# josl/kmerjs

Measured on AMD Instinct MI355X. Metric: k-mers/sec + distinct-kmers/sec, k=16 150bp synthetic FASTQ, 1/2/4/8 GPU, higher is better.
Workload: dtype u8; 1 GPU; C2: 10000000 synthetic 150bp reads per GPU, k=16, prefix 'ATGAC'; reads_per_gpu=10000000, mode=ordered (reference Map insertion order), k=16, prefix=ATGAC, bytes_per_gpu=3170000000, pipeline=off (steps in sequence), parallelism=dp1 (one GPU; no collective), backend=none

## Files before the change

kmerjs_amd/csrc/kmer_kernels.hip:

```cpp
#include "kmer_device.hpp"

#include <algorithm>
#include <cstring>

namespace kmerhip {

__device__ __forceinline__ uint32_t align4(uint32_t hi, uint32_t lo, uint32_t sel) {
    return __builtin_amdgcn_alignbyte(hi, lo, sel);
}

__device__ __forceinline__ void set_info(unsigned int *err, unsigned int bit) {
    if (!(__hip_atomic_load(err, __ATOMIC_RELAXED, __HIP_MEMORY_SCOPE_AGENT) & bit)) atomicOr(err, bit);
}

__device__ __forceinline__ uint32_t not_nl_bits(uint32_t x) {
    return ((x ^ 0x0A0A0A0Au) + 0x7F7F7F7Fu) & 0x80808080u;
}

__device__ __forceinline__ uint32_t not_nl_bits_xad(uint32_t x, uint32_t k0a, uint32_t k7f) {
    uint32_t r;
    asm("v_xad_u32 %0, %1, %2, %3" : "=v"(r) : "v"(x), "v"(k0a), "s"(k7f));
    return r & 0x80808080u;
}

// ... 41 lines not shown
            if (incmask) return acc;
        } else {
            unsigned long long hit = __ballot(inc || val != 0);
            if (hit) {
                int stop = __ffsll((long long)hit) - 1;
                return __shfl(val, stop);
            }
        }
        top -= 64;
    }
}

struct TileShared {
    uint32_t tpre[TPB + 1];
    uint32_t wsum[TPB / 64];
    int32_t last_thr;
    uint32_t tile;
    uint64_t line_base;
    uint64_t lnl_before;
    uint64_t lnl_tile;
    int32_t lastpos;
    uint32_t nh;
    uint32_t qn;
    uint32_t more;
    uint32_t q[1024];
};

__device__ __forceinline__ uint32_t nl_before_in_thread(const uint8_t *buf, int thr, int q) {
    const uint32_t *lw = (const uint32_t *)(buf + FH + 64 * thr);
    int n = q - 64 * thr;
    uint32_t c = 0;
#pragma unroll 1
    for (int i = 0; i < 16 && n > 0; ++i, n -= 4) {
        uint32_t z = nl_flags(lw[i]);
        if (n < 4) z &= (1u << (8 * n)) - 1u;
        c += __popc(z);
    }
    return c;
}

__device__ __forceinline__ uint32_t lds_word(const uint8_t *buf, int p) {
    const int a = FH + p;
    const uint32_t *w = (const uint32_t *)(buf + (a & ~3));
    return align4(w[1], w[0], (uint32_t)(a & 3));
}


__device__ __forceinline__ uint64_t revcomp_code(uint64_t x, uint32_t k) {
    x = ~x;
    x = ((x >> 2) & 0x3333333333333333ull) | ((x & 0x3333333333333333ull) << 2);
    x = ((x >> 4) & 0x0F0F0F0F0F0F0F0Full) | ((x & 0x0F0F0F0F0F0F0F0Full) << 4);
    x = __builtin_bswap64(x);
    return k >= 32 ? x : (x >> (64 - 2 * k));
}

__device__ __forceinline__ void revcomp_code128(uint64_t hi, uint64_t lo, uint32_t k, uint64_t *rhi, uint64_t *rlo) {
    const uint64_t h = revcomp_code(lo, 32), l = revcomp_code(hi, 32);
    const uint32_t s = 128 - 2 * k;
    *rlo = s ? (l >> s) | (h << (64 - s)) : l;
    *rhi = s ? h >> s : h;
}

__device__ __forceinline__ uint32_t tile_prologue(const uint8_t *data, uint64_t len, int64_t g0, uint8_t *buf,
                                                  TileShared &sh, uint32_t (&w)[17], unsigned int *err) {
    const int tid = threadIdx.x, lane = tid & 63, wid = tid >> 6;
    TileRegs r;
    load_tile(data, len, g0, r);
    if (store_tile(r, buf) & 0x80808080u) atomicOr(err, ERR_NONASCII);
    __syncthreads();

    load_thread_words(buf + FH + 64 * tid, w);
    uint32_t cnt = 0;
    const int64_t gt = g0 + 64 * tid;
    if (gt + 64 <= (int64_t)len) {
#pragma unroll
        for (int i = 0; i < 16; ++i) cnt += __popc(nl_flags(w[i]));
    } else {
#pragma unroll
        for (int i = 0; i < 16; ++i) cnt += __popc(nl_flags_below(w[i], (int64_t)len - (gt + 4 * i)));
    }
    uint32_t incl = cnt;
#pragma unroll
    for (int d = 1; d < 64; d <<= 1) {
        const uint32_t y = __shfl_up(incl, d);
        if (lane >= d) incl += y;
    }
    if (lane == 63) sh.wsum[wid] = incl;
    if (cnt) atomicMax(&sh.last_thr, tid);
    __syncthreads();
    uint32_t woff = 0, total = 0;
#pragma unroll
    for (int i = 0; i < TPB / 64; ++i) {
        woff += i < wid ? sh.wsum[i] : 0;
        total += sh.wsum[i];
    }
    sh.tpre[tid] = woff + incl - cnt;
    if (tid == 0) sh.tpre[TPB] = total;
    if (tid == sh.last_thr) {
        int lastpos = -1;
#pragma unroll 1
        for (int i = 15; i >= 0 && lastpos < 0; --i) {
            const uint32_t z = nl_flags_below(*(const uint32_t *)(buf + FH + 64 * tid + 4 * i),
                                              (int64_t)len - (gt + 4 * i));
            if (z) lastpos = 64 * tid + 4 * i + ((31 - __clz(z)) >> 3);
        }
        sh.lastpos = lastpos;
// ... 620 lines not shown
    uint32_t wpre[TPB / 64], wprev[TPB / 64], tcnt = 0, tlast = 0;
    {
        const uint4 ws = *(const uint4 *)sh.wsum, wm = *(const uint4 *)sh.wmax;
        const uint32_t s[4] = {ws.x, ws.y, ws.z, ws.w}, m[4] = {wm.x, wm.y, wm.z, wm.w};
#pragma unroll
        for (int ww = 0; ww < TPB / 64; ++ww) {
            wpre[ww] = tcnt;
            wprev[ww] = tlast;
            tcnt += (uint32_t)__builtin_amdgcn_readfirstlane((int)s[ww]);
            tlast = max(tlast, (uint32_t)__builtin_amdgcn_readfirstlane((int)m[ww]));
        }
    }
    if (tid == 0) {
        a.tsum[tile].cnt = tcnt;
        a.tsum[tile].lnl = tlast ? a.abs_offset + (uint64_t)(g0 + tlast) : 0;
        sh.tcnt = tcnt;
    }
    for (uint32_t done = 0;;) {
        const uint32_t left = total - done;
        uint2 en = make_uint2(0u, 0u);
        if ((uint32_t)tid < min(left, QE)) en = qe[tid];
        const uint32_t nc = __popc(en.y), incl = wave_incl_sum(nc);
        const uint32_t wtot = readlane32(incl, 63);
        uint32_t *flat = sh.flat[wid & 1];
        for (uint32_t cb = 0; cb < wtot; cb += 64) {
            uint32_t m = en.y, p = incl - nc - cb;
            while (m) {
                const uint32_t bit = __ffs(m) - 1;
                m &= m - 1;
                if (p < 64) flat[p] = (en.x + (bit << 1)) | ((uint32_t)tid << 16);
                ++p;
            }
            if ((uint32_t)lane < min(wtot - cb, 64u)) {
                const uint32_t f = flat[lane], ow = (f >> 13) & 3u;
                uint4 lc = sh.qc[f >> 16];
                const uint32_t wp = ow == 0 ? wpre[0] : ow == 1 ? wpre[1] : ow == 2 ? wpre[2] : wpre[3];
                const uint32_t wl = ow == 0 ? wprev[0] : ow == 1 ? wprev[1] : ow == 2 ? wprev[2] : wprev[3];
                const uint32_t prv = lc.x >> 16;
                lc.x = (lc.x & 0xFFFFu) + wp;
                lc.w = prv ? prv : wl;
                emit_hit<true, WIDE, K, PLEN>(a, buf, sh, tile, f & 0xFFFFu, pb, pw, lc, tcnt);
            }
        }
        if (left <= QE) break;
        __syncthreads();
        done += QE;
        enqueue(done);
        __syncthreads();
    }
    if (total > 64) __syncthreads();
    if (tid == 0) put_tile_hits(a, sh, tile);
}

__device__ __forceinline__ uint64_t resolve_hit(const HitArgs &a, uint64_t pos_lines, const HitRec &r,
                                                uint64_t code_hi, const TileSum &tb, uint64_t *order_out,
                                                uint32_t *lk, bool *lvalid_out, uint64_t *key_hi) {
    const uint32_t t = r.tile;
    const uint32_t strand = (r.qm >> 14) & 1u;
    const bool exotic = (r.qm >> 15) & 1u;
    const bool lvalid = (r.qm >> 16) & 1u;
    const int q = (int)(r.qm & 0x3FFFu);
    const int s0 = strand ? q + (int)a.plen - (int)a.k : q;
    const uint64_t tile_abs = a.abs_offset + (uint64_t)t * TILE;
    const uint64_t li = pos_lines + tb.cnt + r.c_local;
    const uint64_t lstart = lvalid ? tile_abs + r.lstart : tb.lnl;
    const uint64_t sabs = tile_abs + (uint64_t)(int64_t)s0;
    uint64_t rel = sabs - lstart;
    const bool seq = (li & 3) == 1;
    const uint64_t maxrel = (1ull << a.pbits) - 1ull;
    if (rel > maxrel) {
        if (seq) atomicOr(a.err, ERR_LINE_TOO_LONG);
        rel = maxrel;
    }
    if (li >> (63 - a.pbits)) atomicOr(a.err, ERR_LINE_TOO_LONG);
    const uint64_t order = (li << (a.pbits + 1)) | ((uint64_t)strand << a.pbits) | (strand ? maxrel - rel : rel);
    *order_out = order;
    const uint32_t sp = (uint32_t)(s0 + 64);
    *lk = (r.c_local << 17) | (strand << 16) | (strand ? 0xFFFFu - sp : sp);
    *lvalid_out = lvalid;
    uint64_t key = a.invalid_key;
    *key_hi = a.wide ? a.invalid_key : 0;
    if (a.wide) key = 0;
    if (seq) {
        if (a.packed && !exotic) {
            if (a.k > 32) {
                uint64_t h = code_hi, l = r.code;
                if (strand) revcomp_code128(code_hi, r.code, a.k, &h, &l);
                key = l & a.smask;
                *key_hi = h & a.smask_hi;
            } else {
                key = (strand ? revcomp_code(r.code, a.k) : r.code) & a.smask;
            }
        } else {
            append_record(a.recs, a.rec_count, a.rec_cap, a.err, order, (uint64_t)t * TILE + (uint64_t)(int64_t)s0, a.k,
                          strand);
        }
    }
    return key;
}

__device__ __forceinline__ void place_hit(const HitArgs &a, uint64_t slot, bool cross, uint64_t xi, uint64_t key,
                                          uint64_t key_hi, uint64_t order) {
    if (!cross) {
        if (slot >= a.rcap) {
            atomicOr(a.err, ERR_OVF_OVERFLOW);
            return;
        }
        if (a.rkey32) a.rkey32[slot] = (uint32_t)key;
        else a.rkey[slot] = key;
        if (a.wide) a.rkeyh[slot] = key_hi;
        a.rord[slot] = order;
    } else if (xi < a.xcap) {
        a.xord[xi] = order;
        a.xslot[xi] = (uint32_t)slot;
        if (a.wide) {
            a.xkey[xi] = xi;
            a.xkeyl[xi] = key;
            a.xkeyh[xi] = key_hi;
        } else {
            a.xkey[xi] = key;
        }
    } else {
        atomicOr(a.err, ERR_CROSS_OVERFLOW);
    }
}

constexpr uint32_t HTPW = 4;
constexpr uint32_t HENT = HTPW * HMAX;
template <bool WIDE>
__global__ __launch_bounds__(256) void hit_kernel(HitArgs a) {
    __shared__ uint32_t s_lk[4][HENT];
    __shared__ uint8_t s_x[4][HENT];
    __shared__ uint64_t s_key[4][HENT];
    __shared__ uint64_t s_ord[4][HENT];
    __shared__ uint64_t s_keyh[WIDE ? 4 : 1][WIDE ? HENT : 1];
    const uint32_t wid = threadIdx.x >> 6, lane = threadIdx.x & 63;
    const uint32_t t0 = __builtin_amdgcn_readfirstlane((blockIdx.x * 4 + wid) * HTPW);
    if (t0 >= a.n_tiles) return;
    const unsigned long long ovf = *a.ovf_count;
    const uint64_t pos_lines = a.pos->lines;
    TileSum ts[HTPW], tb[HTPW];
#pragma unroll
    for (uint32_t u = 0; u < HTPW; ++u) {
        const uint32_t t = min(t0 + u, a.n_tiles - 1);
        ts[u] = a.tsum[t];
        tb[u] = a.tscan[t];
    }
    if (ovf > a.ovf_cap) return;
    uint32_t off[HTPW + 1];
    off[0] = 0;
#pragma unroll
    for (uint32_t u = 0; u < HTPW; ++u) off[u + 1] = off[u] + (t0 + u < a.n_tiles ? min(ts[u].nh, (uint32_t)HMAX) : 0u);
    const uint32_t total = off[HTPW];
    for (uint32_t e0 = 0; e0 < total; e0 += 64) {
        const uint32_t e = e0 + lane;
        if (e < total) {
            uint32_t u = 0;
#pragma unroll
            for (uint32_t v = 1; v < HTPW; ++v) u += e >= off[v] ? 1u : 0u;
            const uint32_t i = e - off[u];
            TileSum tsu = ts[0], tbu = tb[0];
#pragma unroll
            for (uint32_t v = 1; v < HTPW; ++v)
                if (u == v) {
                    tsu = ts[v];
                    tbu = tb[v];
                }
            const uint64_t hslot = (uint64_t)(t0 + u) * HMAX + i;
            const HitRec r = a.hits[hslot];
            uint64_t order, kh;
            uint32_t lk;
            bool lvalid;
            const uint64_t key = resolve_hit(a, pos_lines, r, a.k > 32 ? a.hits_hi[hslot] : 0, tbu, &order, &lk, &lvalid,
                                             &kh);
            s_lk[wid][e] = lk;
            s_x[wid][e] = (tsu.nh > (uint32_t)HMAX || !lvalid || r.c_local == (uint32_t)tsu.cnt) ? 1 : 0;
            s_key[wid][e] = key;
            if (WIDE) s_keyh[WIDE ? wid : 0][WIDE ? e : 0] = kh;
            s_ord[wid][e] = order;
        }
    }
    if (!a.packed) return;
    __builtin_amdgcn_fence(__ATOMIC_RELEASE, "workgroup");
    __builtin_amdgcn_wave_barrier();
    for (uint32_t e0 = 0; e0 < total; e0 += 64) {
        const uint32_t e = e0 + lane;
        if (e >= total) continue;
        uint32_t u = 0;
#pragma unroll
        for (uint32_t v = 1; v < HTPW; ++v) u += e >= off[v] ? 1u : 0u;
        uint32_t lo = off[0], hi = off[1], nh = ts[0].nh;
        uint64_t hb = tb[0].nh, xb = tb[0].nx;
#pragma unroll
        for (uint32_t v = 1; v < HTPW; ++v)
            if (u == v) {
                lo = off[v];
                hi = off[v + 1];
                nh = ts[v].nh;
                hb = tb[v].nh;
                xb = tb[v].nx;
            }
        const uint32_t i = e - lo;
        const bool cross = s_x[wid][e] != 0;
        uint32_t rank = i, xr = i;
        if (nh <= (uint32_t)HMAX) {
            const uint32_t lk = s_lk[wid][e];
            rank = 0;
            xr = 0;
            for (uint32_t j = lo; j < hi; ++j) {
                const uint32_t less = s_lk[wid][j] < lk ? 1u : 0u;
                rank += less;
                xr += less & (uint32_t)s_x[wid][j];
            }
        }
        place_hit(a, a.out_base + hb + rank, cross, a.xbase + xb + xr, s_key[wid][e],
                  WIDE ? s_keyh[WIDE ? wid : 0][WIDE ? e : 0] : 0, s_ord[wid][e]);
    }
}

__global__ __launch_bounds__(256) void hit_overflow_kernel(HitArgs a) {
    const uint64_t n = *a.ovf_count <= a.ovf_cap ? *a.ovf_count : 0;
    for (uint64_t i = (uint64_t)blockIdx.x * blockDim.x + threadIdx.x; i < n; i += (uint64_t)gridDim.x * blockDim.x) {
        const HitRec r = a.ovf[i];
        const TileSum tb = a.tscan[r.tile];
        uint64_t order, kh;
        uint32_t lk;
        bool lvalid;
        const uint64_t key = resolve_hit(a, a.pos->lines, r, a.k > 32 ? a.ovf_hi[i] : 0, tb, &order, &lk, &lvalid, &kh);
        if (!a.packed) continue;
        const uint32_t ord = r.qm >> 17;
        place_hit(a, a.out_base + tb.nh + ord, true, a.xbase + tb.nx + ord, key, kh, order);
    }
    __shared__ bool last;
    __syncthreads();
    if (threadIdx.x == 0) {
        __threadfence();
        last = atomicAdd(a.ticket, 1u) == gridDim.x - 1;
    }
    __syncthreads();
    if (!last || threadIdx.x != 0) return;
    __threadfence();
    const uint32_t nt = a.n_tiles;
    StreamPos *pos = (StreamPos *)a.pos;
    pos->lines += a.tscan[nt - 1].cnt + a.tsum[nt - 1].cnt;
    pos->ends_open = (a.len > 0 && a.data[a.len - 1] != '\n') ? 1 : 0;
    *a.ends_open = pos->ends_open;
    *a.chunk_hits = a.tscan[nt - 1].nh + a.tsum[nt - 1].nh;
    *a.chunk_cross = a.tscan[nt - 1].nx + a.tsum[nt - 1].nx;
    *a.ticket = 0;
    if (a.stamp) a.stamp[STAMP_FEED_END] = wall_clock64();
    const uint64_t errw = __hip_atomic_load(a.scal + 5, __ATOMIC_RELAXED, __HIP_MEMORY_SCOPE_AGENT);
    *a.cross_go = ((uint32_t)errw & CROSS_HOST_BITS) ? 0u : 1u;
    __threadfence();
    if (a.host_out) {
        for (int i = 0; i < 8; ++i)
            a.host_out[i] = i == 5 ? errw : __hip_atomic_load(a.scal + i, __ATOMIC_RELAXED, __HIP_MEMORY_SCOPE_AGENT);
        if (a.stamp)
            for (int i = 0; i <= (int)STAMP_FEED_END; ++i)
                a.host_out[TAIL_STAMP + i] = __hip_atomic_load(a.stamp + i, __ATOMIC_RELAXED, __HIP_MEMORY_SCOPE_AGENT);
        __threadfence_system();
        __hip_atomic_store(a.host_out + 9, a.seq, __ATOMIC_RELEASE, __HIP_MEMORY_SCOPE_SYSTEM);
    }
}

__device__ __forceinline__ TileSum ts_shfl_up(const TileSum &v, int d) {
    TileSum r;
    r.cnt = (uint64_t)__shfl_up((unsigned long long)v.cnt, d);
    r.nh = (uint32_t)__shfl_up((int)v.nh, d);
    r.nx = (uint32_t)__shfl_up((int)v.nx, d);
    r.lnl = (uint64_t)__shfl_up((unsigned long long)v.lnl, d);
    return r;
}
__device__ __forceinline__ TileSum ts_zero() {
    TileSum z;
    z.cnt = 0;
    z.nh = 0;
    z.nx = 0;
    z.lnl = 0;
    return z;
}
__device__ __forceinline__ TileSum ts_wave_scan(TileSum v) {
    const int lane = threadIdx.x & 63;
#pragma unroll
    for (int d = 1; d < 64; d <<= 1) {
// ... 1372 lines not shown
    __shared__ uint32_t cnt[1u << BKT_LOW];
    __shared__ uint32_t s_tot;
    const uint32_t b = blockIdx.x, nk = 1u << shift;
    if (cur && threadIdx.x == 0) s_tot = atomicExch(cur + (uint64_t)b * BKT_CUR_STRIDE, 0u);
    for (uint32_t j = threadIdx.x; j < nk; j += blockDim.x) {
        minr[j] = 0xFFFFFFFFu;
        cnt[j] = 0;
    }
    __syncthreads();
    uint32_t lo, hi;
    if (cur) {
        lo = b * cap;
        hi = s_tot <= cap ? lo + s_tot : lo;
    } else {
        lo = bbase[b];
        hi = bbase[b + 1];
    }
    constexpr uint32_t U = 16;
    for (uint32_t e0 = lo; e0 < hi; e0 += U * 1024) {
        uint32_t j[U], r[U];
#pragma unroll
        for (uint32_t u = 0; u < U; ++u) {
            const uint32_t e = e0 + u * 1024 + threadIdx.x;
            j[u] = e < hi ? pkey[e] & (nk - 1u) : 0u;
            r[u] = e < hi ? prank[e] : 0u;
        }
#pragma unroll
        for (uint32_t u = 0; u < U; ++u) {
            if (e0 + u * 1024 + threadIdx.x < hi) {
                atomicMin(&minr[j[u]], r[u]);
                atomicAdd(&cnt[j[u]], 1u);
            }
        }
    }
    __syncthreads();
    for (uint32_t j = threadIdx.x; j < nk; j += blockDim.x) {
        const uint32_t c = cnt[j];
        if (c) {
            const uint32_t r = minr[j];
            if (r < n) {
                hmark[r] = (uint8_t)min(c, HMARK_FULL);
                if (c >= HMARK_FULL) hcnt[r] = c;
            } else {
                atomicOr(err, ERR_BKT_RANK);
            }
        }
    }
}

constexpr uint32_t EMIT_RPB = 1024;
__global__ __launch_bounds__(256) void head_count_kernel(const uint32_t *hcnt, const uint8_t *hmark, uint64_t n,
                                                         uint32_t *ecnt) {
    __shared__ uint32_t ws[4];
    const uint64_t r0 = (uint64_t)blockIdx.x * EMIT_RPB + 4 * threadIdx.x;
    uint32_t c = 0;
    if (hmark) {
        if (r0 + 4 <= n) {
            const uint32_t v = *(const uint32_t *)(hmark + r0);
            c = ((v & 0xFFu) != 0) + ((v & 0xFF00u) != 0) + ((v & 0xFF0000u) != 0) + ((v & 0xFF000000u) != 0);
        } else {
            for (uint64_t r = r0; r < n; ++r) c += hmark[r] != 0;
        }
    } else if (r0 + 4 <= n) {
        const uint4 v = *(const uint4 *)(hcnt + r0);
        c = (v.x != 0) + (v.y != 0) + (v.z != 0) + (v.w != 0);
    } else {
        for (uint64_t r = r0; r < n; ++r) c += hcnt[r] != 0;
    }
    c = wave_incl_sum(c);
    if ((threadIdx.x & 63) == 63) ws[threadIdx.x >> 6] = c;
    __syncthreads();
    if (threadIdx.x == 0) ecnt[blockIdx.x] = ws[0] + ws[1] + ws[2] + ws[3];
}

__global__ __launch_bounds__(256) void emit_kernel(EmitArgs a) {
    __shared__ __attribute__((aligned(16))) uint8_t kbuf[256 * KMAX_TILE];
    __shared__ uint32_t s_w[EMIT_RPB / 256][4];
    __shared__ uint64_t s_pre;
    __shared__ uint32_t s_wp[4];
    const uint64_t n = a.n;
    const uint32_t k = a.k, plen = a.plen;
    const bool staged = !a.partial && (k & 3);
    const int tid = threadIdx.x, lane = tid & 63, wid = tid >> 6;
    const uint64_t rb = (uint64_t)blockIdx.x * EMIT_RPB;
    constexpr int NR = EMIT_RPB / 256;
    uint32_t hcr[NR];
    unsigned long long hm[NR];
#pragma unroll
    for (int i = 0; i < NR; ++i) {
        const uint64_t r = rb + 256 * i + tid;
        hcr[i] = r < n ? head_count_at(a.hmark, a.hcnt, r) : 0u;
        hm[i] = __ballot(hcr[i] != 0);
        if (lane == 0) s_w[i][wid] = (uint32_t)__popcll(hm[i]);
    }
    uint64_t ekey[NR], ecnt[NR], efirst[NR], ekeyh[NR];
#pragma unroll
    for (int i = 0; i < NR; ++i) {
        const uint64_t r = rb + 256 * i + tid;
        ekey[i] = ecnt[i] = efirst[i] = ekeyh[i] = 0;
        if (hcr[i]) {
            if (a.hrec) {
                const HeadRec v = a.hrec[r];
                ekey[i] = v.key;
                ecnt[i] = v.count;
            } else {
                ekey[i] = a.rkey32 ? (uint64_t)a.rkey32[r] : a.rkey64[r];
                if (a.rkeyh) ekeyh[i] = a.rkeyh[r];
                ecnt[i] = hcr[i];
            }
            efirst[i] = a.rord[r];
        }
    }
    if (a.epre) {
        if (tid == 0) s_pre = a.epre[blockIdx.x];
    } else {
        uint32_t p = 0;
        for (uint32_t j = tid; j < blockIdx.x; j += 256) p += a.ecnt[j];
        p = wave_incl_sum(p);
        if (lane == 63) s_wp[wid] = p;
    }
    __syncthreads();
    if (!a.epre && tid == 0) s_pre = (uint64_t)s_wp[0] + s_wp[1] + s_wp[2] + s_wp[3];
    __syncthreads();
    uint64_t o0 = s_pre;
#pragma unroll
    for (int i = 0; i < NR; ++i) {
        const uint64_t r = rb + 256 * i + tid;
        if (rb + 256 * i >= n) break;
        uint32_t before = 0, rt = 0;
#pragma unroll
        for (int w = 0; w < 4; ++w) {
            before += w < wid ? s_w[i][w] : 0u;
            rt += s_w[i][w];
        }
        const uint32_t hc = hcr[i];
        const uint32_t f = hc ? 1u : 0u;
        const uint64_t o64 = o0 + before +
                             __builtin_amdgcn_mbcnt_hi((uint32_t)(hm[i] >> 32), __builtin_amdgcn_mbcnt_lo((uint32_t)hm[i], 0u));
        const uint64_t oend = o0 + rt;
        if (r == n - 1) {
            *a.nuniq = o64 + f;
            if (a.host_out) {
                a.host_out[TAIL_ERR] = __hip_atomic_load(a.err, __ATOMIC_RELAXED, __HIP_MEMORY_SCOPE_AGENT);
                if (a.stamp) a.host_out[TAIL_FIN_START] = a.stamp[STAMP_FINISH_START];
            }
            if (a.nuniq_host) {
                *a.nuniq_host = o64 + f;
                __threadfence_system();
            }
        }
        const uint64_t o = o64;
        if (f) {
            const uint64_t key = ekey[i], cnt = ecnt[i], keyh = ekeyh[i], first = efirst[i];
            if (a.partial) {
                a.ukey[o] = key;
                Agg v;
                v.first = first;
                v.count = cnt;
                a.uval[o] = v;
            } else {
                a.cnt_out[o] = cnt;
                a.first_out[o] = first;
                uint8_t *out = staged ? kbuf + (o - o0) * k : a.keys_out + o * k;
                const uint32_t nw = (k + 3) / 4;
                uint32_t w0 = 0, w1 = 0, w2 = 0;
                for (int w = 0; w < KMAX_TILE / 4; ++w) {
                    if ((uint32_t)w >= nw) break;
                    uint32_t v = 0;
#pragma unroll
                    for (int j = 0; j < 4; ++j) {
                        const uint32_t pos = 4 * w + j;
                        uint32_t ch = 0;
                        if (pos < plen) {
                            ch = a.P[pos];
                        } else if (pos < k) {
                            const uint32_t sh = 2 * (k - 1 - pos);
                            const uint32_t b = (uint32_t)(sh < 64 ? key >> sh : keyh >> (sh - 64)) & 3u;
                            ch = (0x54474341u >> (8 * b)) & 0xFFu;
                        }
                        v |= ch << (8 * j);
                    }
                    if (k == 16) {
                        if (w == 0) w0 = v;
                        else if (w == 1) w1 = v;
                        else if (w == 2) w2 = v;
                        else *(uint4 *)out = make_uint4(w0, w1, w2, v);
                    } else if ((k & 3) == 0) {
                        *(uint32_t *)(out + 4 * w) = v;
                    } else {
                        for (uint32_t b = 4 * w; b < k && b < 4 * (uint32_t)w + 4; ++b)
                            out[b] = (uint8_t)(v >> (8 * (b & 3)));
                    }
                }
            }
        }
        if (staged) {
            __syncthreads();
            const uint64_t g0 = (uint64_t)o0 * k, g1 = (uint64_t)oend * k;
            const uint64_t a0 = (g0 + 3) & ~3ull, a1 = g1 & ~3ull;
            if (a0 >= a1) {
                for (uint64_t g = g0 + threadIdx.x; g < g1; g += 256) a.keys_out[g] = kbuf[g - g0];
            } else {
                if (threadIdx.x < a0 - g0) a.keys_out[g0 + threadIdx.x] = kbuf[threadIdx.x];
                if (threadIdx.x < g1 - a1) a.keys_out[a1 + threadIdx.x] = kbuf[a1 - g0 + threadIdx.x];
                const uint32_t sh = (uint32_t)(a0 - g0);
                for (uint64_t g = a0 + 4 * threadIdx.x; g < a1; g += 4 * 256) {
                    const uint32_t l = (uint32_t)(g - g0);
                    const uint32_t v = sh == 0 ? *(const uint32_t *)(kbuf + l)
                                               : (uint32_t)kbuf[l] | ((uint32_t)kbuf[l + 1] << 8) |
                                                     ((uint32_t)kbuf[l + 2] << 16) | ((uint32_t)kbuf[l + 3] << 24);
                    *(uint32_t *)(a.keys_out + g) = v;
                }
            }
            __syncthreads();
        }
        o0 = oend;
    }
    if (a.host_out && a.stamp && blockIdx.x == gridDim.x - 1 && tid == 0) {
        a.host_out[TAIL_FIN_END] = wall_clock64();
        __threadfence_system();
    }
}

__global__ __launch_bounds__(256) void merge_prep_kernel(const uint64_t *keys, const Agg *vals, uint64_t n,
                                                         uint64_t *rkey, uint32_t *rkey32, uint64_t *rord,
                                                         uint64_t *rcnt, uint32_t *ridx) {
    for (uint64_t i = (uint64_t)blockIdx.x * blockDim.x + threadIdx.x; i < n; i += (uint64_t)gridDim.x * blockDim.x) {
        const Agg v = vals[i];
        put_key(rkey, rkey32, i, keys[i]);
        rord[i] = v.first;
        rcnt[i] = v.count;
        ridx[i] = (uint32_t)i;
    }
// ... 188 lines not shown
            uint32_t *vw = (uint32_t *)&v;
            for (int j = 0; j < 4; ++j)
                vw[j] = bytes[4 * j] | (bytes[4 * j + 1] << 8) | (bytes[4 * j + 2] << 16) |
                        ((uint32_t)bytes[4 * j + 3] << 24);
            *(uint4 *)(out + o) = v;
        } else {
            for (int b = 0; o + b < total; ++b) out[o + b] = bytes[b];
        }
    }
}

hipError_t launch_lines(const TileArgs &a, bool lookback, hipStream_t s) {
    if (lookback) hipLaunchKernelGGL((lines_kernel<true>), dim3(a.n_tiles), dim3(TPB), 0, s, a);
    else hipLaunchKernelGGL((lines_kernel<false>), dim3(a.n_tiles), dim3(TPB), 0, s, a);
    return hipGetLastError();
}

hipError_t launch_scan_planes(const ScanArgs &a, const PlaneArgs &pa, hipStream_t s) {
    const dim3 g(a.n_tiles);
    uint32_t pm = 0;
    for (int i = 0; i < 5; ++i)
        pm |= (pa.kl[i] ? 1u : 0u) << (4 * i) | (pa.kh[i] ? 1u : 0u) << (4 * i + 1) |
              (pa.rl[i] ? 1u : 0u) << (4 * i + 2) | (pa.rh[i] ? 1u : 0u) << (4 * i + 3);
    if (pa.pb >= 5 && pm == PM_ATGAC) {
        if (a.k == 16 && a.plen == 5)
            hipLaunchKernelGGL((scan_planes_kernel<true, false, PM_ATGAC, 16, 5>), g, dim3(TPB), 0, s, a, pa);
        else if (a.k > 32) hipLaunchKernelGGL((scan_planes_kernel<true, true, PM_ATGAC>), g, dim3(TPB), 0, s, a, pa);
        else hipLaunchKernelGGL((scan_planes_kernel<true, false, PM_ATGAC>), g, dim3(TPB), 0, s, a, pa);
        return hipGetLastError();
    }
    if (a.k > 32) {
        if (pa.pb >= 5) hipLaunchKernelGGL((scan_planes_kernel<true, true>), g, dim3(TPB), 0, s, a, pa);
        else hipLaunchKernelGGL((scan_planes_kernel<false, true>), g, dim3(TPB), 0, s, a, pa);
    } else {
        if (pa.pb >= 5) hipLaunchKernelGGL((scan_planes_kernel<true, false>), g, dim3(TPB), 0, s, a, pa);
        else hipLaunchKernelGGL((scan_planes_kernel<false, false>), g, dim3(TPB), 0, s, a, pa);
    }
    return hipGetLastError();
}
hipError_t launch_scan_tiles(const ScanArgs &a, hipStream_t s) {
    const dim3 g(a.n_tiles);
    if (a.k > 32) {
        if (a.plen >= 4) hipLaunchKernelGGL((scan_tile_kernel<true, true>), g, dim3(TPB), 0, s, a);
        else hipLaunchKernelGGL((scan_tile_kernel<false, true>), g, dim3(TPB), 0, s, a);
    } else {
        if (a.plen >= 4) hipLaunchKernelGGL((scan_tile_kernel<true, false>), g, dim3(TPB), 0, s, a);
        else hipLaunchKernelGGL((scan_tile_kernel<false, false>), g, dim3(TPB), 0, s, a);
    }
    return hipGetLastError();
}

hipError_t launch_hits(const HitArgs &a, hipStream_t s) {
    const dim3 grid((a.n_tiles + 4 * HTPW - 1) / (4 * HTPW));
    if (a.wide) hipLaunchKernelGGL(hit_kernel<true>, grid, dim3(256), 0, s, a);
    else hipLaunchKernelGGL(hit_kernel<false>, grid, dim3(256), 0, s, a);
    hipLaunchKernelGGL(hit_overflow_kernel, dim3(64), dim3(256), 0, s, a);
    return hipGetLastError();
}

hipError_t launch_tile_reduce(const TileSum *in, uint32_t n, TileSum *bsum, uint64_t *stamp, hipStream_t s) {
    hipLaunchKernelGGL(tile_reduce_kernel, dim3((n + TSCAN_BLOCK - 1) / TSCAN_BLOCK), dim3(256), 0, s, in, n, bsum,
                       stamp);
    return hipGetLastError();
}
hipError_t launch_tile_scan(const TileSum *in, uint32_t n, const TileSum *bsum, bool bsum_scanned, TileSum init,
                            TileSum *out, hipStream_t s) {
    hipLaunchKernelGGL(tile_scan_kernel, dim3((n + TSCAN_BLOCK - 1) / TSCAN_BLOCK), dim3(256), 0, s, in, n, bsum,
                       bsum_scanned ? 1u : 0u, init, out);
    return hipGetLastError();
}
hipError_t launch_prep(StreamPos *pos, StreamPos *saved, unsigned int *err, uint64_t *scal, uint32_t flags,
                       uint64_t lines, uint64_t *stamp, hipStream_t s) {
    hipLaunchKernelGGL(prep_kernel, dim3(1), dim3(64), 0, s, pos, saved, err, scal, flags, lines, stamp);
    return hipGetLastError();
}
hipError_t launch_tile_aggregate(const uint8_t *data, uint64_t len, uint32_t n_tiles, uint64_t *agg_cnt,
                                 uint64_t *agg_lnl, unsigned int *err, hipStream_t s) {
    hipLaunchKernelGGL(tile_aggregate_kernel, dim3(n_tiles), dim3(TPB), 0, s, data, len, agg_cnt, agg_lnl, err);
    return hipGetLastError();
}

hipError_t launch_windows(const WindowArgs &a, uint32_t grid, hipStream_t s) {
    hipLaunchKernelGGL(windows_kernel, dim3(grid), dim3(256), 0, s, a);
    return hipGetLastError();
}

static uint32_t grid_for(uint64_t n) {
    uint64_t blocks = (n + 255) / 256;
    if (blocks > 16384) blocks = 16384;
    return (uint32_t)(blocks ? blocks : 1);
}

hipError_t launch_gen_cand(const GenWinArgs &a, const PlaneArgs &pa, hipStream_t s) {
    if (a.len == 0 || a.n_lines == 0) return hipSuccess;
    const uint64_t tiles = (a.len + TILE - 1) / TILE;
    hipLaunchKernelGGL(gen_cand_kernel, dim3((uint32_t)((tiles + GC_TPB - 1) / GC_TPB)), dim3(256), 0, s, a, pa);
    return hipGetLastError();
}

hipError_t launch_gen_fix(const Record *cand, uint64_t n, const SeqLine *lines, uint32_t k, uint32_t plen,
                          uint32_t pbits, Record *recs, unsigned long long *rec_count, uint64_t rec_cap,
                          unsigned int *err, hipStream_t s) {
    if (n == 0) return hipSuccess;
    const uint64_t blocks = std::min<uint64_t>(2048, (n + 4095) / 4096);
    hipLaunchKernelGGL(gen_fix_kernel, dim3((uint32_t)blocks), dim3(256), 0, s, cand, n, lines, k, plen, pbits, recs,
                       rec_count, rec_cap, err);
    return hipGetLastError();
}
// ... 173 lines not shown
        hipLaunchKernelGGL(heads_sparse_kernel<uint32_t>, dim3(grid_for(n)), dim3(256), 0, s, skey32, srank, n,
                           (uint32_t)invalid_key, hcnt);
    else
        hipLaunchKernelGGL(heads_sparse_kernel<uint64_t>, dim3(grid_for(n)), dim3(256), 0, s, skey64, srank, n,
                           invalid_key, hcnt);
    return hipGetLastError();
}
hipError_t launch_heads32(const uint32_t *skey, const uint32_t *srank, uint64_t n, uint32_t invalid_key,
                          const uint64_t *rcnt, HeadRec *hrec, uint32_t *hcnt, hipStream_t s) {
    if (n)
        hipLaunchKernelGGL(heads_kernel<uint32_t>, dim3(grid_for(n)), dim3(256), 0, s, skey, srank, n, invalid_key, rcnt,
                           hrec, hcnt);
    return hipGetLastError();
}
hipError_t launch_bucket_hist(const uint32_t *key, uint64_t n, uint32_t invalid, uint32_t shift, uint32_t nb,
                              uint32_t nblk, uint32_t *H, uint8_t *hmark, uint64_t *stamp, hipStream_t s) {
    hipLaunchKernelGGL(bucket_hist_kernel, dim3(nblk), dim3(256), 0, s, key, n, invalid, shift, nb, nblk, H, hmark,
                       stamp);
    return hipGetLastError();
}
hipError_t launch_bucket_offsets(const uint32_t *H, uint32_t nb, uint32_t nblk, uint32_t *Hs, uint32_t *btot,
                                 uint32_t *bbase, unsigned int *ticket, hipStream_t s) {
    hipLaunchKernelGGL(bucket_offsets_kernel, dim3(nb), dim3(256), 0, s, H, nb, nblk, Hs, btot, bbase, ticket);
    return hipGetLastError();
}
hipError_t launch_bucket_scatter(const uint32_t *key, uint64_t n, uint32_t invalid, uint32_t shift, uint32_t nb,
                                 uint32_t nblk, const uint32_t *Hs, const uint32_t *bbase, uint16_t *pkey,
                                 uint32_t *prank, hipStream_t s) {
    hipLaunchKernelGGL(bucket_scatter_kernel, dim3(nblk), dim3(256), 0, s, key, n, invalid, shift, nb, nblk, Hs, bbase,
                       pkey, prank);
    return hipGetLastError();
}
hipError_t launch_bucket_onepass(const uint32_t *key, uint64_t n, uint32_t invalid, uint32_t shift, uint32_t nb,
                                 uint32_t nblk, uint32_t cap, uint32_t *cur, uint16_t *pkey, uint32_t *prank,
                                 uint8_t *hmark, unsigned int *err, uint64_t *stamp, hipStream_t s) {
    if (nb == 0 || nb > BKT_MAX || (uint64_t)nb * cap > 0x7FFFFFFFull) return hipErrorInvalidValue;
    hipLaunchKernelGGL(bucket_onepass_kernel, dim3(nblk), dim3(256), 0, s, key, n, invalid, shift, nb, cap, cur, pkey,
                       prank, hmark, err, stamp);
    return hipGetLastError();
}
hipError_t launch_bucket_heads(const uint16_t *pkey, const uint32_t *prank, const uint32_t *bbase, uint32_t nb,
                               uint32_t shift, uint8_t *hmark, uint32_t *hcnt, uint32_t *cur, uint32_t cap, uint64_t n,
                               unsigned int *err, hipStream_t s) {
    hipLaunchKernelGGL(bucket_heads_kernel, dim3(nb), dim3(1024), 0, s, pkey, prank, bbase, shift, hmark, hcnt, cur, cap,
                       n, err);
    return hipGetLastError();
}
uint64_t emit_blocks(uint64_t n) { return (n + EMIT_RPB - 1) / EMIT_RPB; }
hipError_t launch_head_count(const uint32_t *hcnt, const uint8_t *hmark, uint64_t n, uint32_t *ecnt, hipStream_t s) {
    if (n) hipLaunchKernelGGL(head_count_kernel, dim3((uint32_t)emit_blocks(n)), dim3(256), 0, s, hcnt, hmark, n, ecnt);
    return hipGetLastError();
}
hipError_t launch_emit(const EmitArgs &a, hipStream_t s) {
    if (a.n) hipLaunchKernelGGL(emit_kernel, dim3((uint32_t)emit_blocks(a.n)), dim3(256), 0, s, a);
    return hipGetLastError();
}
hipError_t launch_merge_prep(const uint64_t *keys, const Agg *vals, uint64_t n, uint64_t *rkey, uint32_t *rkey32,
                             uint64_t *rord, uint64_t *rcnt, uint32_t *ridx, hipStream_t s) {
    if (n)
        hipLaunchKernelGGL(merge_prep_kernel, dim3(grid_for(n)), dim3(256), 0, s, keys, vals, n, rkey, rkey32, rord, rcnt,
                           ridx);
    return hipGetLastError();
}
hipError_t launch_xpart_hist(const uint64_t *rkey, const uint32_t *rkey32, uint64_t n, uint64_t invalid,
                             uint32_t kbits, uint32_t world, uint32_t nblk, uint32_t *H, hipStream_t s) {
    if (world == 0 || world > XP_MAXW || nblk == 0) return hipErrorInvalidValue;
    hipLaunchKernelGGL(xpart_hist_kernel, dim3(nblk), dim3(256), 0, s, rkey, rkey32, n, invalid, kbits, world, nblk, H);
    return hipGetLastError();
}
hipError_t launch_xpart_scatter(const uint64_t *rkey, const uint32_t *rkey32, const uint64_t *rord, uint64_t n,
                                uint64_t invalid, uint32_t kbits, uint32_t world, uint32_t nblk, const uint32_t *H,
                                const uint32_t *Hs, XHit *out, uint64_t *counts, hipStream_t s) {
    if (world == 0 || world > XP_MAXW || nblk == 0) return hipErrorInvalidValue;
    hipLaunchKernelGGL(xpart_scatter_kernel, dim3(nblk), dim3(256), 0, s, rkey, rkey32, rord, n, invalid, kbits, world,
                       nblk, Hs, out);
    hipLaunchKernelGGL(xpart_counts_kernel, dim3(1), dim3(256), 0, s, H, Hs, world, nblk, counts);
    return hipGetLastError();
}
hipError_t launch_xprep(const XHit *x, uint64_t n, uint64_t *rkey, uint32_t *rkey32, uint64_t *rord, uint32_t *ridx,
                        hipStream_t s) {
    if (n) hipLaunchKernelGGL(xprep_kernel, dim3(grid_for(n)), dim3(256), 0, s, x, n, rkey, rkey32, rord, ridx);
    return hipGetLastError();
}
hipError_t launch_gather_records(const Record *recs, uint64_t stride, uint64_t n, const uint8_t *data,
                                 uint8_t *out, hipStream_t s) {
    if (n == 0) return hipSuccess;
    uint64_t blocks = (n + 255) / 256;
    if (blocks > 8192) blocks = 8192;
    hipLaunchKernelGGL(gather_records_kernel, dim3((uint32_t)blocks), dim3(256), 0, s, recs, stride, n, data, out);
    return hipGetLastError();
}

hipError_t launch_nl_write(const uint8_t *data, uint64_t len, uint32_t n_tiles, const uint64_t *tbase, uint64_t *nl,
                           hipStream_t s) {
    hipLaunchKernelGGL(nl_write_kernel, dim3(n_tiles), dim3(256), 0, s, data, len, tbase, nl);
    return hipGetLastError();
}
hipError_t launch_nl_slots(const uint8_t *data, uint64_t len, uint32_t n_tiles, uint32_t cap, uint16_t *slots,
                          uint32_t *tcount, unsigned int *err, hipStream_t s) {
    hipLaunchKernelGGL(nl_slots_kernel, dim3(n_tiles), dim3(256), 0, s, data, len, cap, slots, tcount, err);
    return hipGetLastError();
}
hipError_t launch_seq_lines_slots(const uint16_t *slots, const uint32_t *tcount, const uint64_t *tbase,
                                  uint32_t n_tiles, uint32_t cap, uint64_t len, uint64_t li0, uint64_t first,
                                  uint64_t n_nl, uint64_t n_seq, uint32_t k, uint32_t step, SeqLine *lines,
                                  uint64_t *wcount, unsigned int *err, uint64_t maxrel, hipStream_t s) {
    if (!n_seq) return hipSuccess;
// ... 36 lines not shown
```

Before: 3875 billion k-mers/s.

## Specialize hit and emit kernels for k=16 prefix-5 default shape

Adds compile-time specializations of hit_kernel and emit_kernel for the default k=16, 5-base prefix, narrow-key shape. The specialization uses a 32-bit reverse complement, 32-bit LDS keys, and direct 16-byte k-mer string stores. The hit kernel now loads tile summaries per lane and shares them with ds_bpermute instead of holding per-tile register arrays. It also packs the cross flag into the rank key and vectorises the in-row rank scan with uint4 LDS reads. The head_count kernel is changed to cover a whole EMIT_RPB span per block, and the generic emit path gains a 4-character packed conversion. This adds template variants and tighter bit packing of the local key, at the cost of more code and a risk of overflow in edge cases.

```diff
diff --git a/kmerjs_amd/csrc/kmer_kernels.hip b/kmerjs_amd/csrc/kmer_kernels.hip
--- a/kmerjs_amd/csrc/kmer_kernels.hip
+++ b/kmerjs_amd/csrc/kmer_kernels.hip
@@ -117,6 +117,13 @@
     x = ((x >> 4) & 0x0F0F0F0F0F0F0F0Full) | ((x & 0x0F0F0F0F0F0F0F0Full) << 4);
     x = __builtin_bswap64(x);
     return k >= 32 ? x : (x >> (64 - 2 * k));
+}
+
+__device__ __forceinline__ uint32_t revcomp_code16(uint32_t x) {
+    x = ~x;
+    x = ((x >> 2) & 0x33333333u) | ((x & 0x33333333u) << 2);
+    x = ((x >> 4) & 0x0F0F0F0Fu) | ((x & 0x0F0F0F0Fu) << 4);
+    return __builtin_bswap32(x);
 }
 
 __device__ __forceinline__ void revcomp_code128(uint64_t hi, uint64_t lo, uint32_t k, uint64_t *rhi, uint64_t *rlo) {
@@ -843,68 +850,74 @@
     if (tid == 0) put_tile_hits(a, sh, tile);
 }
 
+template <bool DEF>
 __device__ __forceinline__ uint64_t resolve_hit(const HitArgs &a, uint64_t pos_lines, const HitRec &r,
                                                 uint64_t code_hi, const TileSum &tb, uint64_t *order_out,
                                                 uint32_t *lk, bool *lvalid_out, uint64_t *key_hi) {
+    const uint32_t k = DEF ? 16u : a.k, plen = DEF ? 5u : a.plen, pbits = DEF ? PBITS_DEFAULT : a.pbits;
+    const bool wide = DEF ? false : a.wide != 0, packed = DEF ? true : a.packed != 0;
+    const uint64_t smask = DEF ? (1ull << 22) - 1ull : a.smask, invalid_key = DEF ? 1ull << 22 : a.invalid_key;
     const uint32_t t = r.tile;
     const uint32_t strand = (r.qm >> 14) & 1u;
     const bool exotic = (r.qm >> 15) & 1u;
     const bool lvalid = (r.qm >> 16) & 1u;
     const int q = (int)(r.qm & 0x3FFFu);
-    const int s0 = strand ? q + (int)a.plen - (int)a.k : q;
-    const uint64_t tile_abs = a.abs_offset + (uint64_t)t * TILE;
+    const int s0 = strand ? q + (int)plen - (int)k : q;
     const uint64_t li = pos_lines + tb.cnt + r.c_local;
-    const uint64_t lstart = lvalid ? tile_abs + r.lstart : tb.lnl;
-    const uint64_t sabs = tile_abs + (uint64_t)(int64_t)s0;
-    uint64_t rel = sabs - lstart;
+    uint64_t rel = (uint64_t)(int64_t)(s0 - (int)r.lstart);
+    if (!lvalid) rel = a.abs_offset + (uint64_t)t * TILE + (uint64_t)(int64_t)s0 - tb.lnl;
     const bool seq = (li & 3) == 1;
-    const uint64_t maxrel = (1ull << a.pbits) - 1ull;
+    const uint64_t maxrel = (1ull << pbits) - 1ull;
     if (rel > maxrel) {
         if (seq) atomicOr(a.err, ERR_LINE_TOO_LONG);
         rel = maxrel;
     }
-    if (li >> (63 - a.pbits)) atomicOr(a.err, ERR_LINE_TOO_LONG);
-    const uint64_t order = (li << (a.pbits + 1)) | ((uint64_t)strand << a.pbits) | (strand ? maxrel - rel : rel);
+    if (li >> (63 - pbits)) atomicOr(a.err, ERR_LINE_TOO_LONG);
+    const uint64_t order = (li << (pbits + 1)) | ((uint64_t)strand << pbits) | (strand ? maxrel - rel : rel);
     *order_out = order;
     const uint32_t sp = (uint32_t)(s0 + 64);
-    *lk = (r.c_local << 17) | (strand << 16) | (strand ? 0xFFFFu - sp : sp);
+    *lk = (r.c_local << 16) | (strand << 15) | (strand ? 0x7FFFu - sp : sp);
     *lvalid_out = lvalid;
-    uint64_t key = a.invalid_key;
-    *key_hi = a.wide ? a.invalid_key : 0;
-    if (a.wide) key = 0;
+    uint64_t key = invalid_key;
+    *key_hi = wide ? invalid_key : 0;
+    if (wide) key = 0;
     if (seq) {
-        if (a.packed && !exotic) {
-            if (a.k > 32) {
+        if (packed && !exotic) {
+            if (DEF) {
+                key = (strand ? revcomp_code16((uint32_t)r.code) : (uint32_t)r.code) & (uint32_t)smask;
+            } else if (k > 32) {
                 uint64_t h = code_hi, l = r.code;
-                if (strand) revcomp_code128(code_hi, r.code, a.k, &h, &l);
-                key = l & a.smask;
+                if (strand) revcomp_code128(code_hi, r.code, k, &h, &l);
+                key = l & smask;
                 *key_hi = h & a.smask_hi;
             } else {
-                key = (strand ? revcomp_code(r.code, a.k) : r.code) & a.smask;
+                key = (strand ? revcomp_code(r.code, k) : r.code) & smask;
             }
         } else {
-            append_record(a.recs, a.rec_count, a.rec_cap, a.err, order, (uint64_t)t * TILE + (uint64_t)(int64_t)s0, a.k,
+            append_record(a.recs, a.rec_count, a.rec_cap, a.err, order, (uint64_t)t * TILE + (uint64_t)(int64_t)s0, k,
                           strand);
         }
     }
     return key;
 }
 
+template <bool DEF>
 __device__ __forceinline__ void place_hit(const HitArgs &a, uint64_t slot, bool cross, uint64_t xi, uint64_t key,
                                           uint64_t key_hi, uint64_t order) {
+    const bool wide = DEF ? false : a.wide != 0;
     if (!cross) {
         if (slot >= a.rcap) {
             atomicOr(a.err, ERR_OVF_OVERFLOW);
             return;
         }
-        if (a.rkey32) a.rkey32[slot] = (uint32_t)key;
+        if (DEF || a.rkey32) a.rkey32[slot] = (uint32_t)key;
         else a.rkey[slot] = key;
-        if (a.wide) a.rkeyh[slot] = key_hi;
+        if (wide) a.rkeyh[slot] = key_hi;
         a.rord[slot] = order;
     } else if (xi < a.xcap) {
         a.xord[xi] = order;
         a.xslot[xi] = (uint32_t)slot;
-        if (a.wide) {
+        if (wide) {
             a.xkey[xi] = xi;
             a.xkeyl[xi] = key;
             a.xkeyh[xi] = key_hi;
@@ -918,11 +931,13 @@
 
 constexpr uint32_t HTPW = 4;
 constexpr uint32_t HENT = HTPW * HMAX;
-template <bool WIDE>
+static_assert(HENT * 4 == 64 * 16, "the wave clears its rows with one 16-byte store per lane");
+template <bool WIDE, bool DEF>
 __global__ __launch_bounds__(256) void hit_kernel(HitArgs a) {
-    __shared__ uint32_t s_lk[4][HENT];
-    __shared__ uint8_t s_x[4][HENT];
-    __shared__ uint64_t s_key[4][HENT];
+    static_assert(!(WIDE && DEF), "the default shape has narrow keys");
+    __shared__ __attribute__((aligned(16))) uint32_t s_lk[4][HENT];
+    __shared__ uint64_t s_key[DEF ? 1 : 4][DEF ? 1 : HENT];
+    __shared__ uint32_t s_key32[DEF ? 4 : 1][DEF ? HENT : 1];
     __shared__ uint64_t s_ord[4][HENT];
     __shared__ uint64_t s_keyh[WIDE ? 4 : 1][WIDE ? HENT : 1];
     const uint32_t wid = threadIdx.x >> 6, lane = threadIdx.x & 63;
@@ -930,82 +945,81 @@
     if (t0 >= a.n_tiles) return;
     const unsigned long long ovf = *a.ovf_count;
     const uint64_t pos_lines = a.pos->lines;
-    TileSum ts[HTPW], tb[HTPW];
+    const uint32_t tl = min(t0 + (lane & 3u), a.n_tiles - 1);
+    const TileSum tsl = a.tsum[tl], tbl = a.tscan[tl];
+    ((uint4 *)s_lk[wid])[lane] = make_uint4(~0u, ~0u, ~0u, ~0u);
+    if (ovf > a.ovf_cap) return;
+    const uint32_t nl = t0 + (lane & 3u) < a.n_tiles ? min(tsl.nh, (uint32_t)HMAX) : 0u;
+    uint32_t off[HTPW + 1], nmax = 0;
+    off[0] = 0;
 #pragma unroll
     for (uint32_t u = 0; u < HTPW; ++u) {
-        const uint32_t t = min(t0 + u, a.n_tiles - 1);
-        ts[u] = a.tsum[t];
-        tb[u] = a.tscan[t];
-    }
-    if (ovf > a.ovf_cap) return;
-    uint32_t off[HTPW + 1];
-    off[0] = 0;
-#pragma unroll
-    for (uint32_t u = 0; u < HTPW; ++u) off[u + 1] = off[u] + (t0 + u < a.n_tiles ? min(ts[u].nh, (uint32_t)HMAX) : 0u);
+        const uint32_t nu = readlane32(nl, u);
+        off[u + 1] = off[u] + nu;
+        nmax = max(nmax, nu);
+    }
     const uint32_t total = off[HTPW];
+    auto pull = [](uint32_t u, uint32_t v) { return (uint32_t)__builtin_amdgcn_ds_bpermute((int)(u << 2), (int)v); };
+    auto pull64 = [&](uint32_t u, uint64_t v) {
+        return ((uint64_t)pull(u, (uint32_t)(v >> 32)) << 32) | pull(u, (uint32_t)v);
+    };
     for (uint32_t e0 = 0; e0 < total; e0 += 64) {
         const uint32_t e = e0 + lane;
+        uint32_t u = 0;
+#pragma unroll
+        for (uint32_t v = 1; v < HTPW; ++v) u += e >= off[v] ? 1u : 0u;
+        const uint32_t lo = u == 0 ? off[0] : u == 1 ? off[1] : u == 2 ? off[2] : off[3];
+        const uint32_t nh = pull(u, tsl.nh), cnt = pull(u, (uint32_t)tsl.cnt);
+        TileSum tbu;
+        tbu.cnt = pull64(u, tbl.cnt);
+        tbu.lnl = pull64(u, tbl.lnl);
+        tbu.nh = tbu.nx = 0;
         if (e < total) {
-            uint32_t u = 0;
-#pragma unroll
-            for (uint32_t v = 1; v < HTPW; ++v) u += e >= off[v] ? 1u : 0u;
-            const uint32_t i = e - off[u];
-            TileSum tsu = ts[0], tbu = tb[0];
-#pragma unroll
-            for (uint32_t v = 1; v < HTPW; ++v)
-                if (u == v) {
-                    tsu = ts[v];
-                    tbu = tb[v];
-                }
+            const uint32_t i = e - lo;
             const uint64_t hslot = (uint64_t)(t0 + u) * HMAX + i;
             const HitRec r = a.hits[hslot];
             uint64_t order, kh;
             uint32_t lk;
             bool lvalid;
-            const uint64_t key = resolve_hit(a, pos_lines, r, a.k > 32 ? a.hits_hi[hslot] : 0, tbu, &order, &lk, &lvalid,
-                                             &kh);
-            s_lk[wid][e] = lk;
-            s_x[wid][e] = (tsu.nh > (uint32_t)HMAX || !lvalid || r.c_local == (uint32_t)tsu.cnt) ? 1 : 0;
-            s_key[wid][e] = key;
+            const uint64_t key = resolve_hit<DEF>(a, pos_lines, r, !DEF && a.k > 32 ? a.hits_hi[hslot] : 0, tbu, &order,
+                                                  &lk, &lvalid, &kh);
+            const uint32_t x = (nh > (uint32_t)HMAX || !lvalid || r.c_local == cnt) ? 1u : 0u;
+            s_lk[wid][u * HMAX + i] = (lk << 1) | x;
+            if (DEF) s_key32[DEF ? wid : 0][DEF ? e : 0] = (uint32_t)key;
+            else s_key[DEF ? 0 : wid][DEF ? 0 : e] = key;
             if (WIDE) s_keyh[WIDE ? wid : 0][WIDE ? e : 0] = kh;
             s_ord[wid][e] = order;
         }
     }
-    if (!a.packed) return;
+    if (!DEF && !a.packed) return;
     __builtin_amdgcn_fence(__ATOMIC_RELEASE, "workgroup");
     __builtin_amdgcn_wave_barrier();
     for (uint32_t e0 = 0; e0 < total; e0 += 64) {
         const uint32_t e = e0 + lane;
+        uint32_t u = 0;
+#pragma unroll
+        for (uint32_t v = 1; v < HTPW; ++v) u += e >= off[v] ? 1u : 0u;
+        const uint32_t lo = u == 0 ? off[0] : u == 1 ? off[1] : u == 2 ? off[2] : off[3];
+        const uint32_t nh = pull(u, tsl.nh), hb = pull(u, tbl.nh), xb = pull(u, tbl.nx);
         if (e >= total) continue;
-        uint32_t u = 0;
-#pragma unroll
-        for (uint32_t v = 1; v < HTPW; ++v) u += e >= off[v] ? 1u : 0u;
-        uint32_t lo = off[0], hi = off[1], nh = ts[0].nh;
-        uint64_t hb = tb[0].nh, xb = tb[0].nx;
-#pragma unroll
-        for (uint32_t v = 1; v < HTPW; ++v)
-            if (u == v) {
-                lo = off[v];
-                hi = off[v + 1];
-                nh = ts[v].nh;
-                hb = tb[v].nh;
-                xb = tb[v].nx;
-            }
         const uint32_t i = e - lo;
-        const bool cross = s_x[wid][e] != 0;
-        uint32_t rank = i, xr = i;
-        if (nh <= (uint32_t)HMAX) {
-            const uint32_t lk = s_lk[wid][e];
-            rank = 0;
-            xr = 0;
-            for (uint32_t j = lo; j < hi; ++j) {
-                const uint32_t less = s_lk[wid][j] < lk ? 1u : 0u;
-                rank += less;
-                xr += less & (uint32_t)s_x[wid][j];
-            }
-        }
-        place_hit(a, a.out_base + hb + rank, cross, a.xbase + xb + xr, s_key[wid][e],
-                  WIDE ? s_keyh[WIDE ? wid : 0][WIDE ? e : 0] : 0, s_ord[wid][e]);
+        const uint32_t *row = &s_lk[wid][u * HMAX];
+        const uint32_t lkx = row[i], mine = lkx & ~1u;
+        const bool cross = lkx & 1u;
+        uint32_t acc = 0;
+#pragma clang loop vectorize(disable) unroll(disable)
+        for (uint32_t j = 0; j < nmax; j += 4) {
+            const uint4 w = *(const uint4 *)(row + j);
+            acc += w.x < mine ? (w.x & 1u) | 256u : 0u;
+            acc += w.y < mine ? (w.y & 1u) | 256u : 0u;
+            acc += w.z < mine ? (w.z & 1u) | 256u : 0u;
+            acc += w.w < mine ? (w.w & 1u) | 256u : 0u;
+        }
+        uint32_t rank = acc >> 8, xr = acc & 0xFFu;
+        if (nh > (uint32_t)HMAX) rank = xr = i;
+        place_hit<DEF>(a, a.out_base + hb + rank, cross, a.xbase + xb + xr,
+                       DEF ? (uint64_t)s_key32[DEF ? wid : 0][DEF ? e : 0] : s_key[DEF ? 0 : wid][DEF ? 0 : e],
+                       WIDE ? s_keyh[WIDE ? wid : 0][WIDE ? e : 0] : 0, s_ord[wid][e]);
     }
 }
 
@@ -1017,10 +1031,10 @@
         uint64_t order, kh;
         uint32_t lk;
         bool lvalid;
-        const uint64_t key = resolve_hit(a, a.pos->lines, r, a.k > 32 ? a.ovf_hi[i] : 0, tb, &order, &lk, &lvalid, &kh);
+        const uint64_t key = resolve_hit<false>(a, a.pos->lines, r, a.k > 32 ? a.ovf_hi[i] : 0, tb, &order, &lk, &lvalid, &kh);
         if (!a.packed) continue;
         const uint32_t ord = r.qm >> 17;
-        place_hit(a, a.out_base + tb.nh + ord, true, a.xbase + tb.nx + ord, key, kh, order);
+        place_hit<false>(a, a.out_base + tb.nh + ord, true, a.xbase + tb.nx + ord, key, kh, order);
     }
     __shared__ bool last;
     __syncthreads();
@@ -2499,20 +2513,25 @@
 __global__ __launch_bounds__(256) void head_count_kernel(const uint32_t *hcnt, const uint8_t *hmark, uint64_t n,
                                                          uint32_t *ecnt) {
     __shared__ uint32_t ws[4];
-    const uint64_t r0 = (uint64_t)blockIdx.x * EMIT_RPB + 4 * threadIdx.x;
+    static_assert(EMIT_RPB % 256 == 0, "the emit workgroup's rounds");
+    const uint64_t rb = (uint64_t)blockIdx.x * EMIT_RPB, end = min(n, rb + EMIT_RPB);
     uint32_t c = 0;
-    if (hmark) {
-        if (r0 + 4 <= n) {
-            const uint32_t v = *(const uint32_t *)(hmark + r0);
-            c = ((v & 0xFFu) != 0) + ((v & 0xFF00u) != 0) + ((v & 0xFF0000u) != 0) + ((v & 0xFF000000u) != 0);
+#pragma unroll
+    for (uint32_t p = 0; p < EMIT_RPB; p += 1024) {
+        const uint64_t r0 = rb + p + 4 * threadIdx.x;
+        if (hmark) {
+            if (r0 + 4 <= end) {
+                const uint32_t v = *(const uint32_t *)(hmark + r0);
+                c += ((v & 0xFFu) != 0) + ((v & 0xFF00u) != 0) + ((v & 0xFF0000u) != 0) + ((v & 0xFF000000u) != 0);
+            } else {
+                for (uint64_t r = r0; r < end; ++r) c += hmark[r] != 0;
+            }
+        } else if (r0 + 4 <= end) {
+            const uint4 v = *(const uint4 *)(hcnt + r0);
+            c += (v.x != 0) + (v.y != 0) + (v.z != 0) + (v.w != 0);
         } else {
-            for (uint64_t r = r0; r < n; ++r) c += hmark[r] != 0;
-        }
-    } else if (r0 + 4 <= n) {
-        const uint4 v = *(const uint4 *)(hcnt + r0);
-        c = (v.x != 0) + (v.y != 0) + (v.z != 0) + (v.w != 0);
-    } else {
-        for (uint64_t r = r0; r < n; ++r) c += hcnt[r] != 0;
+            for (uint64_t r = r0; r < end; ++r) c += hcnt[r] != 0;
+        }
     }
     c = wave_incl_sum(c);
     if ((threadIdx.x & 63) == 63) ws[threadIdx.x >> 6] = c;
@@ -2520,14 +2539,30 @@
     if (threadIdx.x == 0) ecnt[blockIdx.x] = ws[0] + ws[1] + ws[2] + ws[3];
 }
 
+
+__device__ __forceinline__ uint32_t acgt4(uint32_t x) {
+    x = (x | (x << 12)) & 0x000F000Fu;
+    x = (x | (x << 6)) & 0x03030303u;
+    return __builtin_bswap32(__builtin_amdgcn_perm(0u, 0x54474341u, x));
+}
+
+__device__ __forceinline__ uint32_t key_bits8(uint64_t key, uint64_t keyh, uint32_t sh) {
+    if (sh >= 64) return (uint32_t)(keyh >> (sh - 64)) & 0xFFu;
+    uint64_t v = key >> sh;
+    if (sh > 56) v |= keyh << (64 - sh);
+    return (uint32_t)v & 0xFFu;
+}
+
+template <bool DEF>
 __global__ __launch_bounds__(256) void emit_kernel(EmitArgs a) {
     __shared__ __attribute__((aligned(16))) uint8_t kbuf[256 * KMAX_TILE];
     __shared__ uint32_t s_w[EMIT_RPB / 256][4];
     __shared__ uint64_t s_pre;
     __shared__ uint32_t s_wp[4];
     const uint64_t n = a.n;
-    const uint32_t k = a.k, plen = a.plen;
-    const bool staged = !a.partial && (k & 3);
+    const uint32_t k = DEF ? 16u : a.k, plen = DEF ? 5u : a.plen;
+    const bool partial = DEF ? false : a.partial != 0;
+    const bool staged = !partial && (k & 3);
     const int tid = threadIdx.x, lane = tid & 63, wid = tid >> 6;
     const uint64_t rb = (uint64_t)blockIdx.x * EMIT_RPB;
     constexpr int NR = EMIT_RPB / 256;
@@ -2545,7 +2580,13 @@
     for (int i = 0; i < NR; ++i) {
         const uint64_t r = rb + 256 * i + tid;
         ekey[i] = ecnt[i] = efirst[i] = ekeyh[i] = 0;
-        if (hcr[i]) {
+        if (DEF) {
+            if (hcr[i]) {
+                ekey[i] = a.rkey32[r];
+                ecnt[i] = hcr[i];
+                efirst[i] = a.rord[r];
+            }
+        } else if (hcr[i]) {
             if (a.hrec) {
                 const HeadRec v = a.hrec[r];
                 ekey[i] = v.key;
@@ -2599,7 +2640,16 @@
         const uint64_t o = o64;
         if (f) {
             const uint64_t key = ekey[i], cnt = ecnt[i], keyh = ekeyh[i], first = efirst[i];
-            if (a.partial) {
+            if (DEF) {
+                a.cnt_out[o] = cnt;
+                a.first_out[o] = first;
+                uint32_t p0, p1;
+                memcpy(&p0, a.P, 4);
+                memcpy(&p1, a.P + 4, 4);
+                const uint32_t c = (uint32_t)key;
+                const uint32_t w1 = (acgt4((c >> 16) & 0x3Fu) & 0xFFFFFF00u) | (p1 & 0xFFu);
+                *(uint4 *)(a.keys_out + o * 16) = make_uint4(p0, w1, acgt4((c >> 8) & 0xFFu), acgt4(c & 0xFFu));
+            } else if (partial) {
                 a.ukey[o] = key;
                 Agg v;
                 v.first = first;
@@ -2614,18 +2664,22 @@
                 for (int w = 0; w < KMAX_TILE / 4; ++w) {
                     if ((uint32_t)w >= nw) break;
                     uint32_t v = 0;
-#pragma unroll
-                    for (int j = 0; j < 4; ++j) {
-                        const uint32_t pos = 4 * w + j;
-                        uint32_t ch = 0;
-                        if (pos < plen) {
-                            ch = a.P[pos];
-                        } else if (pos < k) {
-                            const uint32_t sh = 2 * (k - 1 - pos);
-                            const uint32_t b = (uint32_t)(sh < 64 ? key >> sh : keyh >> (sh - 64)) & 3u;
-                            ch = (0x54474341u >> (8 * b)) & 0xFFu;
+                    if (4 * (uint32_t)w >= plen && 4 * (uint32_t)w + 4 <= k) {
+                        v = acgt4(key_bits8(key, keyh, 2 * (k - 4 - 4 * (uint32_t)w)));
+                    } else {
+#pragma unroll
+                        for (int j = 0; j < 4; ++j) {
+                            const uint32_t pos = 4 * w + j;
+                            uint32_t ch = 0;
+                            if (pos < plen) {
+                                ch = a.P[pos];
+                            } else if (pos < k) {
+                                const uint32_t sh = 2 * (k - 1 - pos);
+                                const uint32_t b = (uint32_t)(sh < 64 ? key >> sh : keyh >> (sh - 64)) & 3u;
+                                ch = (0x54474341u >> (8 * b)) & 0xFFu;
+                            }
+                            v |= ch << (8 * j);
                         }
-                        v |= ch << (8 * j);
                     }
                     if (k == 16) {
                         if (w == 0) w0 = v;
@@ -2920,8 +2974,10 @@
 
 hipError_t launch_hits(const HitArgs &a, hipStream_t s) {
     const dim3 grid((a.n_tiles + 4 * HTPW - 1) / (4 * HTPW));
-    if (a.wide) hipLaunchKernelGGL(hit_kernel<true>, grid, dim3(256), 0, s, a);
-    else hipLaunchKernelGGL(hit_kernel<false>, grid, dim3(256), 0, s, a);
+    const bool def = a.k == 16 && a.plen == 5 && a.packed && a.rkey32 && !a.wide && a.pbits == PBITS_DEFAULT;
+    if (def) hipLaunchKernelGGL((hit_kernel<false, true>), grid, dim3(256), 0, s, a);
+    else if (a.wide) hipLaunchKernelGGL((hit_kernel<true, false>), grid, dim3(256), 0, s, a);
+    else hipLaunchKernelGGL((hit_kernel<false, false>), grid, dim3(256), 0, s, a);
     hipLaunchKernelGGL(hit_overflow_kernel, dim3(64), dim3(256), 0, s, a);
     return hipGetLastError();
 }
@@ -3201,7 +3257,11 @@
     return hipGetLastError();
 }
 hipError_t launch_emit(const EmitArgs &a, hipStream_t s) {
-    if (a.n) hipLaunchKernelGGL(emit_kernel, dim3((uint32_t)emit_blocks(a.n)), dim3(256), 0, s, a);
+    if (!a.n) return hipGetLastError();
+    const dim3 g((uint32_t)emit_blocks(a.n));
+    const bool def = a.k == 16 && a.plen == 5 && !a.partial && !a.hrec && a.rkey32 && !a.rkeyh;
+    if (def) hipLaunchKernelGGL(emit_kernel<true>, g, dim3(256), 0, s, a);
+    else hipLaunchKernelGGL(emit_kernel<false>, g, dim3(256), 0, s, a);
     return hipGetLastError();
 }
 hipError_t launch_merge_prep(const uint64_t *keys, const Agg *vals, uint64_t n, uint64_t *rkey, uint32_t *rkey32,
```

New measurement: 4020 billion k-mers/s (median of 6 runs). +3.7%, better.
